# Baverne/VAE-CYCLEGAN-Implementation

Hardware: AMD Instinct MI355X
Metric: train images/sec (256x256 VAE-CycleGAN step) (higher is better)
Workload: dtype f32; 1 GPU; cyclevaegan unpaired, 3x256x256 synthetic summer<->winter, per-GPU batch 8, latent 64 (BASELINE.json configs[3]/[4]); per_gpu_batch=8, global_batch=8, image_size=256, latent_dim=64, parallelism=dp1, init=random (reference init statistics)

## Files before the change

vae-cyclegan-implementation_amd/csrc/conv_igemm.hip:

```cpp
#include "vcg_common.h"
#ifdef VCG_STAMP
#include <stdlib.h>
#endif

struct ConvP {
  const float* a;
  const float* b;
  const float* bias;
  float* out;
  int N, H, W, Cin, Cout, KH, KW, stride, pad, reflect, ups, act;
  int Hl, Wl, Ho, Wo, M, K;
  int cin4, cout4, cout_log;
  FastDiv fd_howo, fd_wo, fd_cin4, fd_cout4, fd_kw, fd_cin;
  int Hc, Wc, Mc, NB;
  FastDiv fd_hcwc, fd_wc;
  int ktiles_total, sk_len, sk_units, sk_ntn, sk_bm_shift, sk_bn_shift;
  int sk_ntr_pb;
  FastDiv fd_sklen;
  int ksplit, kt_per;
  float* slab;
  int adjoint;
  int src_pitch;
  uint32_t a_bytes, b_bytes;
  int dbl_mirror;
// ... 1773 lines not shown
  Tile out = {64, 64, 1, nkt};
  for (int ci = 0; ci < 5; ++ci) {
    const Cand& c = cands[ci];
    if (c.bn == 32 && !(allow_bn32 && cols <= 32)) continue;
    if (c.bn == 128 && cols <= 64) continue;
    if (c.bm == 128 && rows <= 64) continue;
    const long long tiles = ((rows + c.bm - 1) / c.bm) * ((cols + c.bn - 1) / c.bn) * batches;
    const long long slots = 256LL * c.resident;
    const int max_ns = allow_split ? 32 : 1;
    for (int ns = 1; ns <= max_ns; ++ns) {
      int kt = (nkt + ns - 1) / ns;
      if (ns > 1 && kt < 8) break;
      int real_ns = (nkt + kt - 1) / kt;
      long long rounds = (tiles * real_ns + slots - 1) / slots;
      double t = rounds * kt * c.t_step;
      if (real_ns > 1) t += (double)real_ns * rows * cols * 8.0 / 3.0e6 + 3.0;
      if (t < best * 0.97) { best = t; out = {c.bm, c.bn, real_ns, kt}; }
    }
  }
  return out;
}

static bool wino_takes(const ConvGeom& g, long long gate) {
  const long long kc = (long long)g.ups * g.ups * g.Cin;
  return vcg_wino_weight_ok(g) && kc * g.Cout >= gate * (kc + g.Cout);
}
static bool wino_takes_fwd(const ConvGeom& g) { return wino_takes(g, kWinoGateFwd); }
static bool wino_takes_dgrad(const ConvGeom& g) { return wino_takes(g, kWinoGateDgrad); }
static bool wft_wanted(const ConvGeom& g) { return g.Cout >= 64 && g.Cin % 4 == 0 && !wino_takes_fwd(g); }
static bool wfd_wanted(const ConvGeom& g) {
  return g.Cout >= 64 && g.Cout % 32 == 0 && !wino_takes_dgrad(g) && !vcg_thin_fold_dgrad_ok(g) && !vcg_thin_dgrad_ok(g);
}

struct PackLayout { size_t wf, u, ud, wk, wkd, wft, wfd, hdr, total; };
static PackLayout pack_layout(const ConvGeom& g) {
  PackLayout L;
  size_t o = 0;
  L.wf = o;  o += (((size_t)g.K * g.Cout + 63) / 64) * 64;
  L.u = o;   if (wino_takes_fwd(g)) o += vcg_wino_weight_floats(g);
  L.ud = o;  if (wino_takes_dgrad(g)) o += vcg_wino_weight_floats(g);
  L.wk = o;  if (vcg_thin_fold_ok(g)) o += vcg_thin_fold_weight_floats(g);
  L.wkd = o; if (vcg_thin_fold_dgrad_ok(g)) o += vcg_thin_fold_dgrad_weight_floats(g);
  L.wft = o; if (wft_wanted(g)) o += (size_t)g.Cout * ((g.K + 31) / 32) * VCG_PFLOATS;
  L.wfd = o; if (wfd_wanted(g)) o += (size_t)g.K * (g.Cout / 32) * VCG_PFLOATS;
  L.hdr = o; L.total = o + 16;
  return L;
}

enum FwdPath { FWD_THIN_FOLD, FWD_THIN, FWD_THININ, FWD_WINO, FWD_SLAB, FWD_SPLIT, FWD_FP32 };
struct FwdPlan {
  FwdPath path;
  Tile t;
  bool single_level;
  size_t ws;
  int stats_nchunk;
  size_t part_bytes;
  bool reads_wf;
  bool pre_ok;
  size_t saved_floats;
};
static FwdPlan plan_fwd(const ConvGeom& g) {
  FwdPlan pl = {};
  if (vcg_thin_fold_ok(g)) { pl.path = FWD_THIN_FOLD; pl.ws = vcg_thin_fold_workspace(g); }
  else if (vcg_thin_fwd_ok(g)) { pl.path = FWD_THIN; pl.reads_wf = true; }
  else if (vcg_thinin_fwd_ok(g)) { pl.path = FWD_THININ; pl.reads_wf = true; pl.stats_nchunk = vcg_thinin_nchunk(g); }
  else if (vcg_wino_fwd_ok(g)) {
    pl.path = FWD_WINO; pl.ws = vcg_wino_fwd_workspace(g); pl.pre_ok = true; pl.saved_floats = vcg_wino_saved_floats(g);
    pl.stats_nchunk = (int)(vcg_wino_fwd_stats_doubles(g) / ((size_t)g.N * g.Cout * 2));
  } else if (wft_wanted(g) && vcg_slab_fwd_ok(g)) {
    pl.path = FWD_SLAB;
    if (vcg_slab_fwd_stats_ok(g)) pl.stats_nchunk = vcg_slab_fwd_nchunk(g);
  } else {
    pl.t = gemm_plan(g.M, g.Cout, (g.K + BK - 1) / BK, true, 1, true);
    const bool split = pl.t.bm == 128 && pl.t.bn >= 64 && wft_wanted(g);
    pl.path = split ? FWD_SPLIT : FWD_FP32; pl.single_level = g.K <= 2048; pl.reads_wf = !split;
    if (pl.t.nsplit > 1) pl.ws = (size_t)pl.t.nsplit * g.M * g.Cout * sizeof(float) + 256;
    if (split && pl.t.nsplit == 1 && (g.Ho * g.Wo) % 128 == 0) pl.stats_nchunk = g.Ho * g.Wo / 128;
  }
  pl.part_bytes = pl.stats_nchunk ? (size_t)g.N * pl.stats_nchunk * g.Cout * 2 * sizeof(double)
                                  : vcg_in_workspace(g.N, g.Ho * g.Wo, g.Cout);
  return pl;
}

enum DgradPath { DGRAD_UNSUPPORTED, DGRAD_THIN_FOLD, DGRAD_THIN, DGRAD_WINO, DGRAD_SLAB, DGRAD_SPLIT_PLANES, DGRAD_SPLIT32,
                 DGRAD_SPLIT64_NOPLANES, DGRAD_FP32 };
struct DgradPlan {
  DgradPath path;
  Tile t;
  bool replan;
  size_t ws;
  bool reads_wf;
};
static DgradPlan plan_dgrad(const ConvGeom& g) {
  DgradPlan pl = {};
  const int s = g.stride;
  const bool wfd = wfd_wanted(g);
  if (g.Hl % s || g.Wl % s) { pl.path = DGRAD_UNSUPPORTED; pl.reads_wf = true; }
  else if (vcg_thin_fold_dgrad_ok(g)) { pl.path = DGRAD_THIN_FOLD; pl.ws = vcg_thin_fold_dgrad_workspace(g); }
  else if (vcg_thin_dgrad_ok(g)) { pl.path = DGRAD_THIN; pl.ws = vcg_thin_dgrad_workspace(g); pl.reads_wf = true; }
  else if (vcg_wino_dgrad_ok(g)) { pl.path = DGRAD_WINO; pl.ws = vcg_wino_dgrad_workspace(g); }
  else if (wfd && vcg_slab_dgrad_ok(g)) { pl.path = DGRAD_SLAB; pl.ws = vcg_slab_dgrad_workspace(g); }
  else {
    const int Mc = g.N * (g.Hl / s) * (g.Wl / s), NB = g.ups * g.ups * g.Cin;
    pl.t = gemm_plan(Mc, NB, (g.KH * g.KW * g.Cout + BK - 1) / BK, s == 1, 1, true);
    if (s > 1 && g.KH % s == 0 && g.KW % s == 0) {
      const long long wgs = ((Mc + pl.t.bm - 1) / pl.t.bm) * ((NB + pl.t.bn - 1) / pl.t.bn) * s * s;
      pl.replan = wgs < 384;
      if (pl.replan) pl.t = gemm_plan(Mc, NB, ((g.KH / s) * (g.KW / s) * g.Cout + BK - 1) / BK, true, s * s, true);
    }
    const bool planes = pl.t.bm == 128 && pl.t.bn >= 64 && wfd;
    pl.path = planes ? DGRAD_SPLIT_PLANES : pl.t.bn == 32 ? DGRAD_SPLIT32
              : pl.t.bm == 128 && pl.t.bn == 64 ? DGRAD_SPLIT64_NOPLANES : DGRAD_FP32;
    pl.reads_wf = !planes;
    if (pl.t.nsplit > 1) pl.ws = (size_t)pl.t.nsplit * g.N * g.H * g.W * g.Cin * sizeof(float) + 256;
  }
  return pl;
}

typedef void (*ConvKernel)(ConvP);
struct KernelRef { ConvKernel fn; const char* name; };

static KernelRef fwd_fp32_kernel(const Tile& t, bool single_level) {
  const char* const name = "k_conv_fwd<fp32 MFMA>";
  if (t.bm == 128 && t.bn == 128 && single_level) return {k_conv_fwd<128, 128, 2, false>, name};
  if (t.bn == 32) return {k_conv_fwd<128, 32, 1>, name};
  if (t.bm == 128 && t.bn == 128) return {k_conv_fwd<128, 128>, name};
  if (t.bm == 128 && t.bn == 64) return {k_conv_fwd<128, 64>, name};
  if (t.bm == 64 && t.bn == 128) return {k_conv_fwd<64, 128>, name};
  return {k_conv_fwd<64, 64>, name};
}
static void launch_fwd_tile(const Tile& t, const KernelRef& k, const ConvP& p, hipStream_t st) {
  dim3 grid((p.M + t.bm - 1) / t.bm, (p.Cout + t.bn - 1) / t.bn, p.nbatch * p.ksplit);
  VcgProfScope prof(k.name, 2.0 * p.M * (double)p.K * p.Cout * p.nbatch, st);
  hipLaunchKernelGGL(k.fn, grid, dim3(256), 0, st, p);
}

static ConvGeom gemm_geom(int rows, int K, int Ncols) {
  ConvGeom g = {};
  g.N = 1; g.H = 1; g.W = rows; g.Cin = K; g.Cout = Ncols; g.KH = g.KW = 1; g.stride = 1; g.pad = 0; g.reflect = 0;
  g.ups = 1; g.act = VCG_ACT_NONE; g.cin_log = K; g.cout_log = Ncols;
  g.Hl = 1; g.Wl = rows; g.Ho = 1; g.Wo = rows; g.M = rows; g.K = K; g.taps = 1;
  return g;
}
int vcg_gemm_batched(const float* A, const float* B, float* C, int rows, int K, int Ncols, int batches, hipStream_t st) {
  ConvP p; fill_params(gemm_geom(rows, K, Ncols), p);
  p.a = A; p.b = B; p.bias = nullptr; p.out = C;
  if (set_extents(p, (unsigned long long)rows * K * 4, (unsigned long long)K * Ncols * 4,
                  "vcg_gemm_batched: operand extents must stay below 2 GiB per batch")) return -1;
  p.nbatch = batches; p.a_bstride = (uint32_t)((size_t)rows * K); p.b_bstride = (uint32_t)((size_t)K * Ncols);
  p.out_bstride = (size_t)rows * Ncols;
  VCG_CHECK_ARG((unsigned long long)rows * K * (unsigned long long)batches < (1ull << 32), "vcg_gemm_batched: batch stride overflow");
  const Tile t = gemm_plan(rows, Ncols, (K + BK - 1) / BK, false, batches, false, K <= 2048);
  launch_fwd_tile(t, fwd_fp32_kernel(t, K <= 2048), p, st);
  VCG_LAUNCH_CHECK("vcg_gemm_batched");
  return 0;
}

int vcg_fwd_launch(const ConvGeom& g, const float* x, const float* wf, float* y, hipStream_t st) {
  ConvP p; fill_params(g, p);
  p.a = x; p.b = wf; p.bias = nullptr; p.out = y; p.act = VCG_ACT_NONE;
  if (set_extents(p, (unsigned long long)g.N * g.H * g.W * g.Cin * 4, (unsigned long long)g.K * g.Cout * 4,
                  "vcg_conv_fwd: tensor extents must stay below 2 GiB")) return -1;
  const Tile t = gemm_plan(g.M, g.Cout, (g.K + BK - 1) / BK, false, 1, true);
  launch_fwd_tile(t, fwd_fp32_kernel(t, false), p, st);
  VCG_LAUNCH_CHECK("vcg_conv_fwd(raw)");
  return 0;
}

extern "C" size_t vcg_pack_weight_floats(const int32_t* cd) {
  ConvGeom g;
  if (vcg_conv_geom(cd, &g, "vcg_pack_weight_floats")) return 0;
  return pack_layout(g).total;
}

extern "C" int vcg_pack_weight(const float* w_oihw, float* wf, const int32_t* cd, void* stream) {
  ConvGeom g;
  if (vcg_conv_geom(cd, &g, "vcg_pack_weight")) return -1;
  VCG_CHECK_ARG(w_oihw && wf, "vcg_pack_weight: null pointer");
  const PackLayout L = pack_layout(g);
  hipStream_t st = (hipStream_t)stream;
  const VcgAmaxOut aw = vcg_amax_new(st);
  if (vcg_absmax_launch(w_oihw, (size_t)g.cout_log * g.cin_log * g.ups * g.ups * g.KH * g.KW, aw, st)) return -2;
// ... 133 lines not shown
  ConvGeom g;
  if (vcg_conv_geom(cd, &g, "vcg_conv_fwd_in")) return -1;
  VCG_CHECK_ARG((mean == nullptr) == (rstd == nullptr), "vcg_conv_fwd_in: mean and rstd go together");
  const FwdPlan pl = plan_fwd(g);
  if (!pl.saved_floats) saved = nullptr;
  if (!mean) {
    VCG_CHECK_ARG(ws_bytes >= pl.ws, "vcg_conv_fwd_in: workspace too small (%zu)", ws_bytes);
    return conv_fwd_impl(g, pl, take_fwd_hints(), x, wf, bias, y, ws, ws_bytes, stream, nullptr, nullptr, saved, pre);
  }
  VCG_CHECK_ARG(ws, "vcg_conv_fwd_in: null pointer");
  const size_t cws = up256(pl.ws);
  VCG_CHECK_ARG(ws_bytes >= cws + pl.part_bytes, "vcg_conv_fwd_in: workspace too small (%zu)", ws_bytes);
  double* part = reinterpret_cast<double*>(static_cast<char*>(ws) + cws);
  const bool fused = pl.stats_nchunk > 0;
  const VcgInStatsOut stats = {mean, rstd, g.Ho * g.Wo, eps};
  if (conv_fwd_impl(g, pl, take_fwd_hints(), x, wf, bias, y, ws, cws, stream, fused ? part : nullptr, &stats, saved, pre)) return -1;
  if (fused) return 0;
  return vcg_in_stats_pass(y, mean, rstd, g.N, g.Ho * g.Wo, g.Cout, eps, part, ws_bytes - cws, (hipStream_t)stream);
}
extern "C" int vcg_conv_fwd_in(const float* x, const float* wf, const float* bias, float* y, float* mean, float* rstd,
                               float eps, float* saved, const int32_t* cd, void* ws, size_t ws_bytes, void* stream) {
  return conv_fwd_in_impl(x, wf, bias, y, mean, rstd, eps, saved, cd, ws, ws_bytes, stream, nullptr);
}
extern "C" int vcg_conv_fwd_in_pre(const float* t_prev, const float* pre_mean, const float* pre_rstd, int pre_act, const float* wf,
                                   const float* bias, float* y, float* mean, float* rstd, float eps, float* saved, const int32_t* cd,
                                   void* ws, size_t ws_bytes, void* stream) {
  VCG_CHECK_ARG(pre_mean && pre_rstd, "vcg_conv_fwd_in_pre: null statistics");
  VCG_CHECK_ARG(pre_act >= VCG_ACT_NONE && pre_act <= VCG_ACT_SIGMOID, "vcg_conv_fwd_in_pre: bad activation %d", pre_act);
  const VcgPre pre = {pre_mean, pre_rstd, pre_act};
  (void)vcg_take_hint_x();
  return conv_fwd_in_impl(t_prev, wf, bias, y, mean, rstd, eps, saved, cd, ws, ws_bytes, stream, &pre);
}

extern "C" int vcg_conv_reads_wf(const int32_t* cd) {
  ConvGeom g;
  if (vcg_conv_geom(cd, &g, "vcg_conv_reads_wf")) return 1;
  return (plan_fwd(g).reads_wf || plan_dgrad(g).reads_wf) ? 1 : 0;
}

extern "C" size_t vcg_conv_dgrad_workspace(const int32_t* cd) {
  ConvGeom g;
  if (vcg_conv_geom(cd, &g, "vcg_conv_dgrad_workspace")) return 0;
  return plan_dgrad(g).ws;
}

static KernelRef dgrad_kernel(const DgradPlan& pl) {
  const int bm = pl.t.bm, bn = pl.t.bn;
  if (pl.path == DGRAD_SPLIT_PLANES && bn == 128) return {k_conv_dgrad_split<128, 2>, "k_conv_dgrad_split<128, 2>"};
  if (pl.path == DGRAD_SPLIT_PLANES) return {k_conv_dgrad_split<64, 2>, "k_conv_dgrad_split<64, 2>"};
  if (pl.path == DGRAD_SPLIT32) return {k_conv_dgrad_split<32, 1>, "k_conv_dgrad_split<32, 1>"};
  if (pl.path == DGRAD_SPLIT64_NOPLANES) return {k_conv_dgrad_split<64, 2, false>, "k_conv_dgrad_split<64, 2>"};
  const char* const name = "k_conv_dgrad<fp32 MFMA>";
  if (bn == 32) return {k_conv_dgrad<128, 32, 1>, name};
  if (bm == 128 && bn == 128) return {k_conv_dgrad<128, 128>, name};
  if (bm == 128 && bn == 64) return {k_conv_dgrad<128, 64>, name};
  if (bm == 64 && bn == 128) return {k_conv_dgrad<64, 128>, name};
  return {k_conv_dgrad<64, 64>, name};
}
static void dgrad_setup(const ConvGeom& g, const DgradPlan& pl, void* ws, ConvP& p) {
  p.Hc = g.Hl / g.stride; p.Wc = g.Wl / g.stride; p.Mc = g.N * p.Hc * p.Wc;
  p.NB = g.ups * g.ups * g.Cin;
  p.fd_hcwc = make_fastdiv((uint32_t)(p.Hc * p.Wc));
  p.fd_wc = make_fastdiv((uint32_t)p.Wc);
  auto dbl = [&](int L) { int lo = 1 > L - 1 - g.pad ? 1 : L - 1 - g.pad, hi = g.pad < L - 2 ? g.pad : L - 2; return lo <= hi; };
  p.dbl_mirror = g.reflect && (dbl(g.Hl) || dbl(g.Wl));
  if (pl.t.nsplit > 1) { p.ksplit = pl.t.nsplit; p.kt_per = pl.t.kt_per; p.slab = (float*)ws; }
}

extern "C" int vcg_conv_dgrad(const float* dy, const float* wf, float* dx, const int32_t* cd, void* ws,
                              size_t ws_bytes, void* stream) {
  (void)vcg_take_hint_x();
  const uint64_t dy_handle = vcg_take_hint_dy();
  ConvGeom g;
  if (vcg_conv_geom(cd, &g, "vcg_conv_dgrad")) return -1;
  VCG_CHECK_ARG(dy && wf && dx, "vcg_conv_dgrad: null pointer");
  const DgradPlan pl = plan_dgrad(g);
  VCG_CHECK_ARG(pl.path != DGRAD_UNSUPPORTED, "vcg_conv_dgrad: input %dx%d not divisible by stride", g.Hl, g.Wl);
  VCG_CHECK_ARG(g.stride == 1 || g.ups == 1, "vcg_conv_dgrad: stride 2 with ups 2 unsupported");
  const PackLayout L = pack_layout(g);
  const void* const w_amax = wf + L.hdr;
  hipStream_t st = (hipStream_t)stream;
  if (pl.path == DGRAD_THIN_FOLD) return vcg_thin_fold_dgrad(g, dy, wf + L.wkd, w_amax, dx, ws, ws_bytes, st, dy_handle);
  if (pl.path == DGRAD_THIN) return vcg_thin_dgrad(g, dy, wf, dx, ws, ws_bytes, st);
  if (pl.path == DGRAD_WINO) return vcg_wino_dgrad(g, dy, wf + L.ud, w_amax, dx, ws, ws_bytes, st, dy_handle);
  if (pl.path == DGRAD_SLAB) return vcg_slab_dgrad(g, dy, wf + L.wfd, (L.hdr - L.wfd) * 4, w_amax, dx, ws, ws_bytes, st, dy_handle);
  ConvP p; fill_params(g, p);
  p.a = dy; p.b = wf; p.out = dx;
  if (set_extents(p, (unsigned long long)g.M * g.Cout * 4, (unsigned long long)g.K * g.Cout * 4,
                  "vcg_conv_dgrad: tensor extents must stay below 2 GiB")) return -1;
  const int nsplit = pl.t.nsplit;
  if (nsplit > 1) VCG_CHECK_ARG(ws && ws_bytes >= pl.ws, "vcg_conv_dgrad: workspace too small (%zu)", ws_bytes);
  dgrad_setup(g, pl, ws, p);
  if (pl.path == DGRAD_SPLIT_PLANES) { p.b = wf + L.wfd; p.b_bytes = (uint32_t)((L.hdr - L.wfd) * 4); }
  if (pl.path != DGRAD_FP32) {
    if (vcg_operand_amax(dy, (size_t)g.M * g.Cout, dy_handle, g.reflect ? 4 : 0, st, &p.amax_a)) return -2;
    p.amax_b = vcg_amax_stored(w_amax);
  }
  {
    const KernelRef k = dgrad_kernel(pl);
    dim3 grid((p.Mc + pl.t.bm - 1) / pl.t.bm, (p.NB + pl.t.bn - 1) / pl.t.bn, nsplit * g.stride * g.stride);
    VcgProfScope prof(k.name, 2.0 * g.M * (double)g.K * g.Cout, st);
    hipLaunchKernelGGL(k.fn, grid, dim3(256), 0, st, p);
  }
  if (nsplit > 1)
    hipLaunchKernelGGL(k_splitk_finish, dim3(ew_grid((size_t)g.N * g.H * g.W * g.Cin / 4)), dim3(256), 0, st,
                       (const float*)ws, (const float*)nullptr, dx, (size_t)g.N * g.H * g.W, g.Cin, nsplit, g.Cin,
                       (int)VCG_ACT_NONE);
  VCG_LAUNCH_CHECK("vcg_conv_dgrad");
  return 0;
}

struct WgradPlan { int bm, bn, grid, len, parts, total, ntr, ntn; };
static WgradPlan wgrad_plan(const ConvGeom& g, int batches = 1) {
  WgradPlan best_p = {};
  const int total = (g.M + BK - 1) / BK;
  struct Cand { int bm, bn, resident; double t_step; };
  const Cand cands[4] = {{256, 128, 1, 4.3}, {128, 128, 2, 5.1}, {128, 64, 3, 4.7}, {64, 64, 5, 4.8}};
  double best = 1e30;
  int force = 0;
#ifdef VCG_STAMP
  { const char* e = getenv("VCG_WGRAD_BM"); force = e ? atoi(e) : 0; }
#endif
  for (int ci = 0; ci < 4; ++ci) {
    const Cand& c = cands[ci];
    if (force ? c.bm != force : c.bm == 256) continue;
    if (c.bn == 128 && g.Cout <= 64) continue;
    if (c.bm >= 128 && g.K <= 64) continue;
    if (c.bm == 256 && g.K < 512) continue;
    if (batches > 1 && g.K % c.bm) continue;
    const int ntr = ((g.K + c.bm - 1) / c.bm) * batches, ntn = (g.Cout + c.bn - 1) / c.bn;
    const long long tiles = (long long)ntr * ntn, units = tiles * total;
    if (units >= (1LL << 30)) continue;
    const long long slots = 256LL * c.resident;
    long long len = (units + slots - 1) / slots;
    if (len < 8) len = units < 8 ? units : 8;
    const long long grid = (units + len - 1) / len;
    const int parts = (int)((total + len - 1) / len) + 1;
    double t = (double)len * c.t_step + (double)(grid + tiles) * c.bm * c.bn * 8.0 / 3.0e6;
    if (t < best * 0.97) {
      best = t;
      best_p = {c.bm, c.bn, (int)grid, (int)len, parts, total, ntr, ntn};
    }
  }
  return best_p;
}

static void stream_k_setup(const WgradPlan& wp, ConvP& p) {
  p.ktiles_total = wp.total; p.sk_len = wp.len; p.sk_units = wp.ntr * wp.ntn * wp.total; p.sk_ntn = wp.ntn;
  p.sk_bm_shift = wp.bm == 256 ? 8 : wp.bm == 128 ? 7 : 6; p.sk_bn_shift = wp.bn == 128 ? 7 : 6;
  p.fd_sklen = make_fastdiv((uint32_t)wp.len);
}
static void launch_stream_k(const WgradPlan& wp, const ConvP& p, double flops, hipStream_t st) {
  const int bm = wp.bm, bn = wp.bn;
  const KernelRef k = bm == 128 && bn == 128  ? KernelRef{k_conv_wgrad_split<128>, "k_conv_wgrad_split<128>"}
                      : bm == 128 && bn == 64 ? KernelRef{k_conv_wgrad_split<64>, "k_conv_wgrad_split<64>"}
                      : bm == 64 && bn == 128 ? KernelRef{k_conv_wgrad<64, 128>, "k_conv_wgrad<fp32 MFMA>"}
                      : bm == 64              ? KernelRef{k_conv_wgrad<64, 64>, "k_conv_wgrad<fp32 MFMA>"}
                                              : KernelRef{k_conv_wgrad<256, 128, 512>, "k_conv_wgrad<fp32 MFMA>"};
  VcgProfScope prof(k.name, flops, st);
  hipLaunchKernelGGL(k.fn, dim3(wp.grid), dim3(bm == 256 ? 512 : 256), 0, st, p);
}

static const int kMaxDirectSlabs = 24;

static void colsum_plan(const ConvGeom& g, int& tc, int& cgroups, int& rows, int& nchunk) {
  int c4 = g.Cout / 4;
// ... 180 lines not shown
```

vae-cyclegan-implementation_amd/csrc/conv_thinin.hip:

```cpp
#include "vcg_common.h"

struct ThinInP {
  const float* x;
  const float* wf;
  const float* bias;
  float* y;
  double* in_part;
  int N, H, W, Ho, Wo, Cout, cout_log, pad, reflect, act, nbx, nby;
  VcgAmax amax_a, amax_b;
};

template <int KH, int KW, int S>
__global__ __launch_bounds__(256, 2) void k_conv_thinin(ThinInP p) {
  constexpr int SH = 15 * S + KH, SW = 15 * S + 8, SPX = SH * SW;
  constexpr int BN = 64;
  __shared__ __attribute__((aligned(16))) unsigned char As[VCG_NP][SPX * 8];
  __shared__ __attribute__((aligned(16))) unsigned char Bs[VCG_NP][KH * 4 * BN * 16];
  __shared__ double red[4 * BN * 2];
  const int tid = threadIdx.x, lane = tid & 63, wid = tid >> 6, l31 = lane & 31, lh = lane >> 5;
  float sA, invA, sB, invB;
  vcg_scale_of(vcg_amax_bits(p.amax_a), p.amax_a.shift, sA, invA);
  vcg_scale_of(vcg_amax_bits(p.amax_b), p.amax_b.shift, sB, invB);
  int blk = blockIdx.x;
  const int n = blk / (p.nbx * p.nby);
// ... 67 lines not shown
  int abase[2];
#pragma unroll
  for (int i = 0; i < 2; ++i) {
    const int m = wid * 64 + i * 32 + l31;
    abase[i] = ((m >> 4) * S) * SW + (m & 15) * S;
  }
#pragma unroll 1
  for (int kh = 0; kh < KH; ++kh) {
#pragma unroll
    for (int ks = 0; ks < 2; ++ks) {
      const int chunk = ks * 2 + lh;
      f16x8 a[VCG_NP][2], b[VCG_NP][2];
#pragma unroll
      for (int pc = 0; pc < VCG_NP; ++pc) {
#pragma unroll
        for (int i = 0; i < 2; ++i) {
          const uint32_t o = (uint32_t)((abase[i] + kh * SW + 2 * chunk) * 8);
          const uint2 q0 = *reinterpret_cast<const uint2*>(&As[pc][o]);
          const uint2 q1 = *reinterpret_cast<const uint2*>(&As[pc][o + 8]);
          const uint4 q = make_uint4(q0.x, q0.y, q1.x, q1.y);
          a[pc][i] = __builtin_bit_cast(f16x8, q);
        }
#pragma unroll
        for (int j = 0; j < 2; ++j)
          b[pc][j] = *reinterpret_cast<const f16x8*>(&Bs[pc][(uint32_t)(((kh * 4 + chunk) * BN + j * 32 + l31) * 16)]);
      }
#pragma unroll
      for (int i = 0; i < 2; ++i)
#pragma unroll
        for (int j = 0; j < 2; ++j) {
          f32x16 c = lo[i][j];
          c = VCG_MFMA(a[1][i], b[0][j], c);
          c = VCG_MFMA(a[0][i], b[1][j], c);
          lo[i][j] = c;
          acc[i][j] = VCG_MFMA(a[0][i], b[0][j], acc[i][j]);
        }
    }
  }

  const float oscale = sA * sB;
#pragma unroll
  for (int j = 0; j < 2; ++j) {
    const int co = j * 32 + l31;
    const float bv = (p.bias && co < p.cout_log) ? p.bias[co] : 0.f;
    double s1 = 0.0, s2 = 0.0;
#pragma unroll
    for (int i = 0; i < 2; ++i) {
#pragma unroll
      for (int e = 0; e < 16; ++e) {
        const int row = (e & 3) + 8 * (e >> 2) + 4 * lh;
        const int m = wid * 64 + i * 32 + row;
        const int oy = oy0 + (m >> 4), ox = ox0 + (m & 15);
        const float v = act_apply((acc[i][j][e] + lo[i][j][e]) * oscale + bv, p.act);
        if (co < p.Cout) p.y[(((size_t)n * p.Ho + oy) * p.Wo + ox) * p.Cout + co] = v;
        s1 += (double)v;
        s2 += (double)v * (double)v;
      }
    }
    if (p.in_part) {
      s1 += __shfl_xor(s1, 32);
      s2 += __shfl_xor(s2, 32);
      if (lh == 0) {
        red[(wid * BN + co) * 2] = s1;
        red[(wid * BN + co) * 2 + 1] = s2;
      }
    }
  }
  if (p.in_part) {
    __syncthreads();
    if (tid < BN && tid < p.Cout) {
      double t1 = 0.0, t2 = 0.0;
#pragma unroll
      for (int w = 0; w < 4; ++w) {
        t1 += red[(w * BN + tid) * 2];
        t2 += red[(w * BN + tid) * 2 + 1];
      }
      double* o = p.in_part + (((size_t)n * (p.nbx * p.nby) + blk) * p.Cout + tid) * 2;
      o[0] = t1;
      o[1] = t2;
    }
  }
}

bool vcg_thinin_fwd_ok(const ConvGeom& g) {
  return g.KH == 4 && g.KW == 4 && g.stride == 2 && g.pad == 1 && g.ups == 1 && g.Cin == 4 && g.Cout == 64 && g.Ho % 16 == 0 &&
         g.Wo % 16 == 0 && g.Ho > 0 && g.Wo > 0 && (!g.reflect || (g.H > g.pad + 8 && g.W > g.pad + 8));
}
int vcg_thinin_nchunk(const ConvGeom& g) { return (g.Ho / 16) * (g.Wo / 16); }
int vcg_thinin_fwd(const ConvGeom& g, const float* x, const float* wf, const void* w_amax, const float* bias, float* y, double* in_part,
                   hipStream_t st, uint64_t x_handle) {
  ThinInP p = {};
  if (vcg_operand_amax(x, (size_t)g.N * g.H * g.W * g.Cin, x_handle, 0, st, &p.amax_a)) return -2;
  p.amax_b = vcg_amax_stored(w_amax);
  p.x = x; p.wf = wf; p.bias = bias; p.y = y; p.in_part = in_part;
  p.N = g.N; p.H = g.H; p.W = g.W; p.Ho = g.Ho; p.Wo = g.Wo; p.Cout = g.Cout; p.cout_log = g.cout_log;
  p.pad = g.pad; p.reflect = g.reflect; p.act = g.act; p.nbx = g.Wo / 16; p.nby = g.Ho / 16;
  const dim3 grid((unsigned)(g.N * p.nbx * p.nby));
  const double flops = 2.0 * g.M * (double)g.K * g.Cout;
  {
    VcgProfScope prof("k_conv_thinin<4, 4, 2>", flops, st);
    hipLaunchKernelGGL((k_conv_thinin<4, 4, 2>), grid, dim3(256), 0, st, p);
  }
  VCG_LAUNCH_CHECK("vcg_conv_fwd(thin input)");
  return 0;
}
```

vae-cyclegan-implementation_amd/csrc/vcg_common.h:

```cpp
#pragma once
#include <hip/hip_runtime.h>
#include <stdint.h>
#include <stdio.h>
#include <string.h>
#include "../../include/vcg.h"

#define VCG_WAVE 64

typedef float f32x16 __attribute__((ext_vector_type(16)));
typedef float f32x4 __attribute__((ext_vector_type(4)));

void vcg_set_error(const char* fmt, ...);

#define VCG_CHECK_ARG(cond, ...)      \
  do {                                \
    if (!(cond)) {                    \
      vcg_set_error(__VA_ARGS__);     \
      return -1;                      \
    }                                 \
  } while (0)

#define VCG_LAUNCH_CHECK(name)                                              \
  do {                                                                      \
    hipError_t e__ = hipGetLastError();                                     \
// ... 166 lines not shown
    uint32_t m = red[0];
    for (int w = 1; w < nw; ++w) m = red[w] > m ? red[w] : m;
    atomicMax(slot + (blockIdx.x & 63), ((unsigned long long)gen << 32) | m);
  }
}
__device__ __forceinline__ uint32_t vcg_abs_bits(float v) { return __float_as_uint(v) & 0x7FFFFFFFu; }
__device__ __forceinline__ uint32_t vcg_abs_bits4(const float4& v) {
  const uint32_t a = vcg_abs_bits(v.x), b = vcg_abs_bits(v.y), c = vcg_abs_bits(v.z), d = vcg_abs_bits(v.w);
  const uint32_t ab = a > b ? a : b, cd = c > d ? c : d;
  return ab > cd ? ab : cd;
}
__device__ __forceinline__ uint32_t vcg_amax_bits(const VcgAmax& a) {
  if (!a.slot) return a.stored ? *a.stored : a.bits;
  const unsigned long long w = a.slot[threadIdx.x & 63];
  uint32_t b = (uint32_t)(w >> 32) == a.gen ? (uint32_t)w : 0u;
#pragma unroll
  for (int o = 32; o > 0; o >>= 1) {
    const uint32_t other = (uint32_t)__shfl_xor((int)b, o, 64);
    b = other > b ? other : b;
  }
  return b;
}
#endif
__host__ __device__ static inline void vcg_scale_of(uint32_t amax_bits, int shift, float& s, float& inv) {
  int e = (int)((amax_bits >> 23) & 0xFF);
  int f = (e == 0 || e == 255) ? 127 + shift : e - 14 + shift;
  f = f < 1 ? 1 : (f > 253 ? 253 : f);
  const uint32_t sb = (uint32_t)f << 23, ib = (uint32_t)(254 - f) << 23;
#ifdef __HIP_DEVICE_COMPILE__
  s = __uint_as_float(sb); inv = __uint_as_float(ib);
#else
  memcpy(&s, &sb, 4); memcpy(&inv, &ib, 4);
#endif
}

struct NormPlan {
  int TC, TP, cgroups, nchunk, chunk;
};
static inline NormPlan vcg_norm_plan(int N, int HW, int C) {
  NormPlan pl;
  int c4 = C / 4;
  int tc = 1;
  while (tc * 2 <= c4 && tc * 2 <= 32) tc *= 2;
  pl.TC = tc;
  pl.TP = 256 / tc;
  pl.cgroups = (c4 + tc - 1) / tc;
  long long target = 1024 / ((long long)N * pl.cgroups);
  if (target < 1) target = 1;
  long long maxc = (HW + pl.TP * 2 - 1) / (pl.TP * 2);
  if (maxc < 1) maxc = 1;
  if (target > maxc) target = maxc;
  pl.chunk = (int)((HW + target - 1) / target);
  pl.nchunk = (HW + pl.chunk - 1) / pl.chunk;
  return pl;
}
int vcg_in_finalize(const double* part, float* mean, float* rstd, int N, int HW, int C, int nchunk, float eps, hipStream_t st);

struct VcgInStatsOut {
  float* mean;
  float* rstd;
  int HW;
  float eps;
};
int vcg_in_stats_pass(const float* t, float* mean, float* rstd, int N, int HW, int C, float eps, void* ws, size_t ws_bytes, hipStream_t st);

struct ConvGeom {
  int N, H, W, Cin, Cout, KH, KW, stride, pad, reflect, ups, act, cin_log, cout_log;
  int Hl, Wl, Ho, Wo, M, K, taps;
};

int vcg_conv_geom(const int32_t* cd, ConvGeom* g, const char* who);

bool vcg_thin_fwd_ok(const ConvGeom& g);
bool vcg_thin_dgrad_ok(const ConvGeom& g);
size_t vcg_thin_dgrad_workspace(const ConvGeom& g);
int vcg_thin_fwd(const ConvGeom& g, const float* x, const float* wf, const float* bias, float* y, hipStream_t st);
int vcg_thin_dgrad(const ConvGeom& g, const float* dy, const float* wf, float* dx, void* ws, size_t ws_bytes,
                   hipStream_t st);

bool vcg_thinin_fwd_ok(const ConvGeom& g);
int vcg_thinin_nchunk(const ConvGeom& g);
int vcg_thinin_fwd(const ConvGeom& g, const float* x, const float* wf, const void* w_amax, const float* bias, float* y, double* in_part,
                   hipStream_t st, uint64_t x_handle);

bool vcg_wino_weight_ok(const ConvGeom& g);
constexpr long long kWinoGateFwd = 100, kWinoGateDgrad = 80, kWinoGateWgrad = 128;
bool vcg_wino_fwd_ok(const ConvGeom& g);
size_t vcg_wino_weight_floats(const ConvGeom& g);
size_t vcg_wino_fwd_workspace(const ConvGeom& g);
int vcg_wino_weight(const ConvGeom& g, const float* w_oihw, float* u, const VcgAmax& amax_w, hipStream_t st);
struct VcgPre { const float* mean; const float* rstd; int act; };
int vcg_wino_fwd(const ConvGeom& g, const float* x, const float* u, const void* w_amax, const float* bias, float* y, void* ws,
                 size_t ws_bytes, hipStream_t st, double* in_part = nullptr, const VcgInStatsOut* stats = nullptr, float* v_keep = nullptr,
                 uint64_t x_handle = 0, const VcgPre* pre = nullptr);
size_t vcg_wino_saved_floats(const ConvGeom& g);
size_t vcg_wino_fwd_stats_doubles(const ConvGeom& g);
bool vcg_wino_wgrad_ok(const ConvGeom& g);
size_t vcg_wino_wgrad_workspace(const ConvGeom& g);
int vcg_wino_wgrad(const ConvGeom& g, const float* x, const float* dy, float* gw_oihw, void* ws, size_t ws_bytes, hipStream_t st,
                   const float* v_saved = nullptr, uint64_t x_handle = 0, uint64_t dy_handle = 0);
bool vcg_wino_wgrad_tr_ok(const ConvGeom& g);
int vcg_wino_wgrad_reduce_one(const ConvGeom& g, const float* dU, float* gw_oihw, hipStream_t st);
size_t vcg_wino_wgrad_core_workspace(const ConvGeom& g, int T);
int vcg_wino_wgrad_core(const ConvGeom& g, const float* V, const float* dM, int T, float* gw_oihw, void* ws, size_t ws_bytes,
                        hipStream_t st, const VcgAmax& amax_v, const VcgAmax& amax_dm);
bool vcg_wino_dgrad_ok(const ConvGeom& g);
size_t vcg_wino_dgrad_workspace(const ConvGeom& g);
int vcg_wino_weight_dgrad(const ConvGeom& g, const float* w_oihw, float* ud, const VcgAmax& amax_w, hipStream_t st);
int vcg_wino_dgrad(const ConvGeom& g, const float* dy, const float* ud, const void* w_amax, float* dx, void* ws, size_t ws_bytes,
                   hipStream_t st, uint64_t dy_handle = 0);
bool vcg_slab_fwd_ok(const ConvGeom& g);
bool vcg_slab_fwd_stats_ok(const ConvGeom& g);
int vcg_slab_fwd_nchunk(const ConvGeom& g);
bool vcg_slab_dgrad_ok(const ConvGeom& g);
size_t vcg_slab_dgrad_workspace(const ConvGeom& g);
int vcg_slab_fwd(const ConvGeom& g, const float* x, const void* wft_planes, size_t planes_bytes, const void* w_amax, const float* bias,
                 float* y, double* in_part, const VcgInStatsOut* stats, hipStream_t st, uint64_t x_handle = 0);
int vcg_slab_dgrad(const ConvGeom& g, const float* dy, const void* wfd_planes, size_t planes_bytes, const void* w_amax, float* dx,
                   void* ws, size_t ws_bytes, hipStream_t st, uint64_t dy_handle = 0);
bool vcg_ring_wgrad_ok(const ConvGeom& g);
size_t vcg_ring_wgrad_workspace(const ConvGeom& g);
int vcg_ring_wgrad(const ConvGeom& g, const float* x, const float* dy, float* gw_oihw, void* ws, size_t ws_bytes, hipStream_t st,
                   uint64_t x_handle = 0, uint64_t dy_handle = 0);
bool vcg_thin_fold_ok(const ConvGeom& g);
size_t vcg_thin_fold_weight_floats(const ConvGeom& g);
size_t vcg_thin_fold_workspace(const ConvGeom& g);
int vcg_thin_fold_pack(const ConvGeom& g, const float* w_oihw, float* wk, const VcgAmax& amax_w, hipStream_t st);
int vcg_thin_fold_fwd(const ConvGeom& g, const float* x, const float* wk, const void* w_amax, const float* bias, float* y, void* ws,
                      size_t ws_bytes, hipStream_t st, uint64_t x_handle = 0);
bool vcg_thin_fold_dgrad_ok(const ConvGeom& g);
size_t vcg_thin_fold_dgrad_weight_floats(const ConvGeom& g);
size_t vcg_thin_fold_dgrad_workspace(const ConvGeom& g);
int vcg_thin_fold_dgrad_pack(const ConvGeom& g, const float* w_oihw, float* wk, const VcgAmax& amax_w, hipStream_t st);
int vcg_thin_fold_dgrad(const ConvGeom& g, const float* dy, const float* wkd, const void* w_amax, float* dx, void* ws, size_t ws_bytes,
                        hipStream_t st, uint64_t dy_handle = 0);
```

Before: 257.2 images/s.

## Add dedicated dgrad kernel for thin-input 4x4 stride-2 convolution

Adds a specialized input-gradient kernel for the 4-channel-input, 64-output 4x4 stride-2 conv, used in the discriminator's first layer. It computes per-output-pixel tap products with split-f16 MFMA against all 16 taps x 4 channels, stages them in LDS, then gathers the overlapping tap contributions, including reflect-pad folding, into dx. This replaces the generic split/implicit-GEMM dgrad path, which handles the tiny Cin=4 output dimension poorly. The cost is recomputing the halo pixels that neighbouring tiles overlap, and extra LDS traffic.

```diff
diff --git a/vae-cyclegan-implementation_amd/csrc/conv_igemm.hip b/vae-cyclegan-implementation_amd/csrc/conv_igemm.hip
--- a/vae-cyclegan-implementation_amd/csrc/conv_igemm.hip
+++ b/vae-cyclegan-implementation_amd/csrc/conv_igemm.hip
@@ -1879,7 +1879,7 @@
   return pl;
 }
 
-enum DgradPath { DGRAD_UNSUPPORTED, DGRAD_THIN_FOLD, DGRAD_THIN, DGRAD_WINO, DGRAD_SLAB, DGRAD_SPLIT_PLANES, DGRAD_SPLIT32,
+enum DgradPath { DGRAD_UNSUPPORTED, DGRAD_THIN_FOLD, DGRAD_THIN, DGRAD_THININ, DGRAD_WINO, DGRAD_SLAB, DGRAD_SPLIT_PLANES, DGRAD_SPLIT32,
                  DGRAD_SPLIT64_NOPLANES, DGRAD_FP32 };
 struct DgradPlan {
   DgradPath path;
@@ -1895,6 +1895,7 @@
   if (g.Hl % s || g.Wl % s) { pl.path = DGRAD_UNSUPPORTED; pl.reads_wf = true; }
   else if (vcg_thin_fold_dgrad_ok(g)) { pl.path = DGRAD_THIN_FOLD; pl.ws = vcg_thin_fold_dgrad_workspace(g); }
   else if (vcg_thin_dgrad_ok(g)) { pl.path = DGRAD_THIN; pl.ws = vcg_thin_dgrad_workspace(g); pl.reads_wf = true; }
+  else if (vcg_thinin_dgrad_ok(g)) { pl.path = DGRAD_THININ; pl.reads_wf = true; }
   else if (vcg_wino_dgrad_ok(g)) { pl.path = DGRAD_WINO; pl.ws = vcg_wino_dgrad_workspace(g); }
   else if (wfd && vcg_slab_dgrad_ok(g)) { pl.path = DGRAD_SLAB; pl.ws = vcg_slab_dgrad_workspace(g); }
   else {
@@ -2194,6 +2195,7 @@
   hipStream_t st = (hipStream_t)stream;
   if (pl.path == DGRAD_THIN_FOLD) return vcg_thin_fold_dgrad(g, dy, wf + L.wkd, w_amax, dx, ws, ws_bytes, st, dy_handle);
   if (pl.path == DGRAD_THIN) return vcg_thin_dgrad(g, dy, wf, dx, ws, ws_bytes, st);
+  if (pl.path == DGRAD_THININ) return vcg_thinin_dgrad(g, dy, wf, w_amax, dx, st, dy_handle);
   if (pl.path == DGRAD_WINO) return vcg_wino_dgrad(g, dy, wf + L.ud, w_amax, dx, ws, ws_bytes, st, dy_handle);
   if (pl.path == DGRAD_SLAB) return vcg_slab_dgrad(g, dy, wf + L.wfd, (L.hdr - L.wfd) * 4, w_amax, dx, ws, ws_bytes, st, dy_handle);
   ConvP p; fill_params(g, p);
diff --git a/vae-cyclegan-implementation_amd/csrc/conv_thinin.hip b/vae-cyclegan-implementation_amd/csrc/conv_thinin.hip
--- a/vae-cyclegan-implementation_amd/csrc/conv_thinin.hip
+++ b/vae-cyclegan-implementation_amd/csrc/conv_thinin.hip
@@ -173,6 +173,137 @@
   }
 }
 
+struct ThinInDgradP {
+  const float* dy;
+  const float* wf;
+  float* dx;
+  int N, H, W, Ho, Wo, reflect, nbx, nby;
+  VcgAmax amax_a, amax_b;
+};
+
+#define TD_AROW 144
+#define TD_PROW 68
+
+__global__ __launch_bounds__(256, 2) void k_thinin_dgrad(ThinInDgradP p) {
+  constexpr int C = 64;
+  __shared__ __attribute__((aligned(16))) unsigned char lds[VCG_NP * 256 * TD_AROW];
+  unsigned char* const As0 = lds;
+  unsigned char* const As1 = lds + 256 * TD_AROW;
+  float* const Ps = reinterpret_cast<float*>(lds);
+  const int tid = threadIdx.x, lane = tid & 63, wid = tid >> 6, l31 = lane & 31, lh = lane >> 5;
+  float sA, invA, sB, invB;
+  vcg_scale_of(vcg_amax_bits(p.amax_a), p.amax_a.shift, sA, invA);
+  vcg_scale_of(vcg_amax_bits(p.amax_b), p.amax_b.shift, sB, invB);
+  int blk = blockIdx.x;
+  const int n = blk / (p.nbx * p.nby);
+  blk -= n * p.nbx * p.nby;
+  const int by = blk / p.nbx, bx = blk - by * p.nbx;
+  const int a0 = by * 15 - 1, b0 = bx * 15 - 1;
+
+  const float* dyn = p.dy + (size_t)n * p.Ho * p.Wo * C;
+#pragma unroll
+  for (int half = 0; half < 2; ++half) {
+    float4 v[8];
+#pragma unroll
+    for (int r = 0; r < 8; ++r) {
+      const int it = tid + 256 * (half * 8 + r);
+      const int px = it >> 4, q = it & 15;
+      const int oh = a0 + (px >> 4), ow = b0 + (px & 15);
+      const bool ok = oh >= 0 && oh < p.Ho && ow >= 0 && ow < p.Wo;
+      v[r] = ok ? *reinterpret_cast<const float4*>(dyn + ((size_t)oh * p.Wo + ow) * C + q * 4) : make_float4(0.f, 0.f, 0.f, 0.f);
+    }
+#pragma unroll
+    for (int r = 0; r < 8; ++r) {
+      const int it = tid + 256 * (half * 8 + r);
+      const int px = it >> 4, q = it & 15;
+      uint2 h, l;
+      split4h(v[r], invA, h, l);
+      *reinterpret_cast<uint2*>(As0 + px * TD_AROW + q * 8) = h;
+      *reinterpret_cast<uint2*>(As1 + px * TD_AROW + q * 8) = l;
+    }
+  }
+  f16x8 b[VCG_NP][2][4];
+#pragma unroll
+  for (int j = 0; j < 2; ++j)
+#pragma unroll
+    for (int ks = 0; ks < 4; ++ks) {
+      const float* q = p.wf + (size_t)(j * 32 + l31) * C + ks * 16 + lh * 8;
+      const float4 w0 = *reinterpret_cast<const float4*>(q), w1 = *reinterpret_cast<const float4*>(q + 4);
+      uint2 h0, l0, h1, l1;
+      split4h(w0, invB, h0, l0);
+      split4h(w1, invB, h1, l1);
+      b[0][j][ks] = __builtin_bit_cast(f16x8, make_uint4(h0.x, h0.y, h1.x, h1.y));
+      b[1][j][ks] = __builtin_bit_cast(f16x8, make_uint4(l0.x, l0.y, l1.x, l1.y));
+    }
+  __syncthreads();
+
+  f32x16 acc[2][2], lo[2][2];
+#pragma unroll
+  for (int i = 0; i < 2; ++i)
+#pragma unroll
+    for (int j = 0; j < 2; ++j)
+#pragma unroll
+      for (int e = 0; e < 16; ++e) acc[i][j][e] = lo[i][j][e] = 0.f;
+#pragma unroll
+  for (int ks = 0; ks < 4; ++ks) {
+    f16x8 a[VCG_NP][2];
+#pragma unroll
+    for (int i = 0; i < 2; ++i) {
+      const uint32_t o = (uint32_t)((wid * 64 + i * 32 + l31) * TD_AROW + ks * 32 + lh * 16);
+      a[0][i] = *reinterpret_cast<const f16x8*>(As0 + o);
+      a[1][i] = *reinterpret_cast<const f16x8*>(As1 + o);
+    }
+#pragma unroll
+    for (int i = 0; i < 2; ++i)
+#pragma unroll
+      for (int j = 0; j < 2; ++j) {
+        f32x16 c = lo[i][j];
+        c = VCG_MFMA(a[1][i], b[0][j][ks], c);
+        c = VCG_MFMA(a[0][i], b[1][j][ks], c);
+        lo[i][j] = c;
+        acc[i][j] = VCG_MFMA(a[0][i], b[0][j][ks], acc[i][j]);
+      }
+  }
+  __syncthreads();
+
+  const float oscale = sA * sB;
+#pragma unroll
+  for (int i = 0; i < 2; ++i)
+#pragma unroll
+    for (int j = 0; j < 2; ++j)
+#pragma unroll
+      for (int e = 0; e < 16; ++e) {
+        const int row = wid * 64 + i * 32 + (e & 3) + 8 * (e >> 2) + 4 * lh;
+        Ps[row * TD_PROW + j * 32 + l31] = (acc[i][j][e] + lo[i][j][e]) * oscale;
+      }
+  __syncthreads();
+
+  float* dxn = p.dx + (size_t)n * p.H * p.W * 4;
+  for (int idx = tid; idx < 900; idx += 256) {
+    const int lr = idx / 30, lc = idx - lr * 30;
+    const int h = by * 30 - 1 + lr, w = bx * 30 - 1 + lc;
+    if (h < 0 || h >= p.H || w < 0 || w >= p.W) continue;
+    int rs[3], cs[3], nr = 2, nc = 2;
+    rs[0] = (lr >> 1) * 16 * TD_PROW + (2 + (lr & 1)) * 16;
+    rs[1] = ((lr >> 1) + 1) * 16 * TD_PROW + (lr & 1) * 16;
+    cs[0] = (lc >> 1) * TD_PROW + (2 + (lc & 1)) * 4;
+    cs[1] = ((lc >> 1) + 1) * TD_PROW + (lc & 1) * 4;
+    if (p.reflect) {
+      if (h == 1) rs[nr++] = (lr >> 1) * 16 * TD_PROW;
+      if (h == p.H - 2) rs[nr++] = ((lr >> 1) + 1) * 16 * TD_PROW + 3 * 16;
+      if (w == 1) cs[nc++] = (lc >> 1) * TD_PROW;
+      if (w == p.W - 2) cs[nc++] = ((lc >> 1) + 1) * TD_PROW + 3 * 4;
+    }
+    float4 s = make_float4(0.f, 0.f, 0.f, 0.f);
+    for (int a = 0; a < nr; ++a)
+      for (int c = 0; c < nc; ++c) {
+        const float4 t = *reinterpret_cast<const float4*>(Ps + rs[a] + cs[c]);
+        s.x += t.x; s.y += t.y; s.z += t.z; s.w += t.w;
+      }
+    *reinterpret_cast<float4*>(dxn + ((size_t)h * p.W + w) * 4) = s;
+  }
+}
+
 bool vcg_thinin_fwd_ok(const ConvGeom& g) {
   return g.KH == 4 && g.KW == 4 && g.stride == 2 && g.pad == 1 && g.ups == 1 && g.Cin == 4 && g.Cout == 64 && g.Ho % 16 == 0 &&
          g.Wo % 16 == 0 && g.Ho > 0 && g.Wo > 0 && (!g.reflect || (g.H > g.pad + 8 && g.W > g.pad + 8));
@@ -195,3 +326,24 @@
   VCG_LAUNCH_CHECK("vcg_conv_fwd(thin input)");
   return 0;
 }
+
+bool vcg_thinin_dgrad_ok(const ConvGeom& g) {
+  return g.KH == 4 && g.KW == 4 && g.stride == 2 && g.pad == 1 && g.ups == 1 && g.Cin == 4 && g.Cout == 64 && g.H % 2 == 0 &&
+         g.W % 2 == 0 && (long long)g.H * g.W >= 64 * 64;
+}
+int vcg_thinin_dgrad(const ConvGeom& g, const float* dy, const float* wf, const void* w_amax, float* dx, hipStream_t st,
+                     uint64_t dy_handle) {
+  ThinInDgradP p = {};
+  if (vcg_operand_amax(dy, (size_t)g.M * g.Cout, dy_handle, 0, st, &p.amax_a)) return -2;
+  p.amax_b = vcg_amax_stored(w_amax);
+  p.dy = dy; p.wf = wf; p.dx = dx;
+  p.N = g.N; p.H = g.H; p.W = g.W; p.Ho = g.Ho; p.Wo = g.Wo; p.reflect = g.reflect;
+  p.nbx = (g.W + 1 + 29) / 30; p.nby = (g.H + 1 + 29) / 30;
+  const dim3 grid((unsigned)(g.N * p.nbx * p.nby));
+  {
+    VcgProfScope prof("k_thinin_dgrad<4, 4, 2>", 2.0 * g.M * (double)g.K * g.Cout, st);
+    hipLaunchKernelGGL(k_thinin_dgrad, grid, dim3(256), 0, st, p);
+  }
+  VCG_LAUNCH_CHECK("vcg_conv_dgrad(thin input)");
+  return 0;
+}
diff --git a/vae-cyclegan-implementation_amd/csrc/vcg_common.h b/vae-cyclegan-implementation_amd/csrc/vcg_common.h
--- a/vae-cyclegan-implementation_amd/csrc/vcg_common.h
+++ b/vae-cyclegan-implementation_amd/csrc/vcg_common.h
@@ -272,6 +272,9 @@
 int vcg_thinin_nchunk(const ConvGeom& g);
 int vcg_thinin_fwd(const ConvGeom& g, const float* x, const float* wf, const void* w_amax, const float* bias, float* y, double* in_part,
                    hipStream_t st, uint64_t x_handle);
+bool vcg_thinin_dgrad_ok(const ConvGeom& g);
+int vcg_thinin_dgrad(const ConvGeom& g, const float* dy, const float* wf, const void* w_amax, float* dx, hipStream_t st,
+                     uint64_t dy_handle);
 
 bool vcg_wino_weight_ok(const ConvGeom& g);
 constexpr long long kWinoGateFwd = 100, kWinoGateDgrad = 80, kWinoGateWgrad = 128;
```

After: 257.1 images/s, median of 2. Within noise of the previous version (-0.0%).
